# bobu36000/gym-chess

Hardware: AMD Instinct MI355X
Metric: env steps/sec at 65 536 boards per GPU (random-policy self-play to terminal, auto-reset) (higher is better)
Workload: dtype u64

## Files before the change

### __graft_entry__.py

```python
import os
import subprocess
import sys

ROOT = os.path.dirname(os.path.abspath(__file__))
PKG_DIR = os.path.join(ROOT, "gym-chess_amd")
LIB = os.path.join(PKG_DIR, "gym_chess_amd", "libgymchess.so")
CORE_HOST = os.path.join(ROOT, "tests", "core_host")


def _run(cmd):
    print("+", " ".join(cmd), flush=True)
    subprocess.run(cmd, check=True)


def _lib_module():
    sys.path.insert(0, PKG_DIR)
    from gym_chess_amd import _lib

    return _lib


def build_hip(force=False):
    L = _lib_module()
    want = L.source_hash()
    if not force and os.path.exists(LIB) and L.built_hash(LIB) == want:
        return
    tmp = LIB + ".tmp"
    _run(["hipcc"] + L.BUILD_FLAGS + [f'-DGC_SRC_HASH="{want}"', "-o", tmp,
                                      os.path.join(PKG_DIR, "csrc", "gymchess.hip")])
    os.replace(tmp, LIB)


def build_oracle():
    _run(["make", "-s", "-C", os.path.join(ROOT, "oracle")])


def build_core_host():
    sys.path.insert(0, CORE_HOST)
    import applysplithost
    import clonehost
    import corehost
    import minimaxhost
    import playouthost
    import quiescehost
    import rankfillhost
    import sworiginhost

    corehost.ensure_built()
    sworiginhost.ensure_built()
    rankfillhost.ensure_built()
    clonehost.ensure_built()
    applysplithost.ensure_built()
    playouthost.ensure_built()
    minimaxhost.ensure_built()
    quiescehost.ensure_built()


def build():
    build_hip()
    build_oracle()
    build_core_host()
    sys.path.insert(0, PKG_DIR)
    import gym_chess_amd
    from gym_chess_amd import _lib

    _lib.load()


def smoke():
    sys.path.insert(0, PKG_DIR)
    sys.path.insert(0, os.path.join(ROOT, "oracle"))
    import numpy as np

    import oracle as O
    from gym_chess_amd.engine import Engine
    from gym_chess_amd.env import BatchedChessEnv

    eng = Engine(0)
    b = np.tile(O.DEFAULT_BOARD, (64, 1))
    m = np.tile(O.make_meta(), (64, 1))
    nodes = eng.perft(b, m, 3)
    assert (nodes == 8982).all(), nodes[:4]
    moves, cnt = eng.possible_moves(b[:1], m[:1], True)
    assert [int(x) for x in moves[0, : cnt[0]]] == O.get_possible_moves(O.DEFAULT_BOARD, O.make_meta(), True)
    env = BatchedChessEnv(32, device=0, seed=7)
    _, tr = env.rollout(60, trace=True)
    for i in range(32):
        ref = O.rollout_trace(7, i, 60)
        assert (tr["action"][:, i] == ref["action"]).all(), f"board {i} actions differ"
        assert (tr["reward"][:, i] == ref["reward"]).all(), f"board {i} rewards differ"
        assert (tr["done"][:, i] == ref["done"]).all(), f"board {i} done differs"
    print("smoke ok: perft(3)=8982 x64, startpos list, 32x60-ply rollout == oracle", flush=True)


if __name__ == "__main__":
    build()
    if len(sys.argv) > 1 and sys.argv[1] == "smoke":
        smoke()
```

### gym-chess_amd/csrc/gc_core.h

```cpp
#pragma once
#include <type_traits>
#include <stdint.h>

#if defined(__HIPCC__)
#include <hip/hip_runtime.h>
#define GC_HD __host__ __device__ __forceinline__
#define GC_HDM __host__ __device__ __forceinline__
#else
#define GC_HD static inline
#define GC_HDM inline
#endif

namespace gc {

typedef uint64_t u64;
typedef uint32_t u32;

enum { EMPTY = 0, KING = 1, QUEEN = 2, ROOK = 3, BISHOP = 4, KNIGHT = 5, PAWN = 6 };
enum { A_KSW = 4096, A_QSW = 4097, A_KSB = 4098, A_QSB = 4099, A_RESIGN = 4100, A_NONE = 0xFFFF };

enum : u32 {
    M_WHITE = 1u, M_WKC = 2u, M_WQC = 4u, M_BKC = 8u, M_BQC = 16u, M_RIGHTS = 30u,
    M_WCHK = 32u, M_BCHK = 64u, M_DONE = 128u,
    M_MC_SHIFT = 8, M_MC_MASK = 0xFFu << 8,
// ... 1047 lines not shown
        if (k >= cc) { k -= cc; v >>= w; base += w; }
    }
    return base;
}
GC_HD u64 fast_pawn_targets(const MoveSet& ms, int sq, bool white) {
    u64 m = bit(sq);
    u64 t1 = white ? ((ms.o1 & m) >> 8) : ((ms.o1 & m) << 8);
    u64 t2 = white ? ((ms.o2 & m) >> 16) : ((ms.o2 & m) << 16);
    u64 tl = white ? ((ms.ol & m) >> 7) : ((ms.ol & m) << 9);
    u64 tr = white ? ((ms.orr & m) >> 9) : ((ms.orr & m) << 7);
    return t1 | t2 | tl | tr;
}
template <class S>
GC_HD int select_action(const Pos& s, const Gen& g, const MoveSet& ms, const S& scr, int k) {
    int normal = ms.total - popc(g.castles);
    if (k >= normal) {
        k -= normal;
        if (g.castles & 2) { if (k == 0) return g.white ? A_KSW : A_KSB; k--; }
        return g.white ? A_QSW : A_QSB;
    }
    if (ms.big) {
        u64 pcs = g.own;
        while (pcs) {
            int sq = ctz(pcs);
            pcs ^= bit(sq);
            u64 tg = legal_targets(s, g, sq, type_at(s, sq));
            int c = popc(tg);
            if (k < c) return sq * 64 + kth_set_bit(tg, k);
            k -= c;
        }
        return A_NONE;
    }
    int lo = 0, pre = 0;
#pragma unroll
    for (int step = 32; step; step >>= 1) {
        int p = prefix_count(ms.cnt, below(lo + step));
        bool take = p <= k;
        lo = take ? lo + step : lo;
        pre = take ? p : pre;
    }
    k -= pre;
    u64 parked = scr.get(ordinal(g.own, lo));
    u64 tg = ((ms.fastp >> lo) & 1) ? fast_pawn_targets(ms, lo, g.white) : parked;
    return lo * 64 + kth_set_bit(tg, k);
}

GC_HD u64 byte_popc(u64 x) {
    x = x - ((x >> 1) & 0x5555555555555555ull);
    x = (x & 0x3333333333333333ull) + ((x >> 2) & 0x3333333333333333ull);
    return (x + (x >> 4)) & 0x0F0F0F0F0F0F0F0Full;
}
GC_HD u64 spread8(u32 b) {
    u64 y = ((u64)(b & 0xFFu) * 0x0101010101010101ull) & 0x8040201008040201ull;
    return ((y + 0x7F7F7F7F7F7F7F7Full) >> 7) & 0x0101010101010101ull;
}
GC_HD int first_byte_above(u64 p, int k) {
    int r = (int)((p >> 24) & 0xFF) <= k ? 4 : 0;
    r += (int)((p >> (8 * r + 8)) & 0xFF) <= k ? 2 : 0;
    r += (int)((p >> (8 * r)) & 0xFF) <= k ? 1 : 0;
    return r;
}
template <class S>
GC_HD int select_action_swar(const Pos& s, const Gen& g, const MoveSet& ms, const S& scr, int k) {
    const int normal = ms.total - popc(g.castles);
    if (k >= normal || ms.big || normal > 255) return select_action(s, g, ms, scr, k);
    const u64 rows = byte_popc(ms.cnt[0]) + (byte_popc(ms.cnt[1]) << 1) + (byte_popc(ms.cnt[2]) << 2) +
                     (byte_popc(ms.cnt[3]) << 3) + (byte_popc(ms.cnt[4]) << 4);
    const u64 rpre = rows * 0x0101010101010101ull;
    const int r = first_byte_above(rpre, k);
    k -= r ? (int)((rpre >> (8 * r - 8)) & 0xFF) : 0;
    const int sh = 8 * r;
    const u64 sqs = spread8((u32)(ms.cnt[0] >> sh)) + (spread8((u32)(ms.cnt[1] >> sh)) << 1) +
                    (spread8((u32)(ms.cnt[2] >> sh)) << 2) + (spread8((u32)(ms.cnt[3] >> sh)) << 3) +
                    (spread8((u32)(ms.cnt[4] >> sh)) << 4);
    const u64 spre = sqs * 0x0101010101010101ull;
    const int f = first_byte_above(spre, k);
    k -= f ? (int)((spre >> (8 * f - 8)) & 0xFF) : 0;
    const int lo = sh + f;
    u64 parked = scr.get(ordinal(g.own, lo));
    u64 tg = ((ms.fastp >> lo) & 1) ? fast_pawn_targets(ms, lo, g.white) : parked;
    return lo * 64 + kth_set_bit(tg, k);
}

GC_HD int sw_origin(const Gen& g, int j, int to) {
    const u64 w0 = g.white ? pack8(8, 16, 7, 9, -15, -17, 17, 15) : pack8(-8, -16, -9, -7, -15, -17, 17, 15);
    const u64 w1 = pack8(-6, -10, 10, 6, 0, 0, 0, 0), w2 = pack8(0, 0, 0, 0, 8, -8, 1, -1);
    const u64 w3 = pack8(9, 7, -7, -9, 0, 0, 0, 0);
    const int q = j >> 3;
    const u64 w = q == 0 ? w0 : q == 1 ? w1 : q == 2 ? w2 : w3;
    const int off = (int)(signed char)(w >> (8 * (j & 7)));
    const int d = (j - SW_ORTH) & 7;
    const bool up = ((0xC6u >> d) & 1) != 0;
    const bool file = d < 2, row = d < 4, dg = d == 5 || d == 6;
    const u64 pl = file ? 0x0080808080808080ull : row ? 0x7FFFFFFFFFFFFFFFull : dg ? 0x0040201008040201ull : 0x0102040810204081ull;
    const u64 ph = file ? 0x0101010101010100ull : row ? 0xFFFFFFFFFFFFFFFEull : dg ? 0x8040201008040200ull : 0x8102040810204080ull;
    const u64 x = g.occ & (up ? pl >> (63 - to) : ph << to);
    const int sl = x ? (up ? msb(x) : ctz(x)) : 0;
    const bool slider = j >= SW_ORTH && j < SW_K;
    return slider ? sl : to + off;
}
GC_HD int sw_select(const Gen& g, const u64* t, int k) {
    int j = SW_SETS;
    u64 tj = 0;
#pragma unroll
    for (int i = 0; i < SW_SETS; i++) {
        const int c = popc(t[i]);
        const bool hit = j == SW_SETS && k < c;
        j = hit ? i : j;
        tj = hit ? t[i] : tj;
        k = j == SW_SETS ? k - c : k;
    }
    if (j == SW_SETS) {
        if ((g.castles & 1) && k == 0) return g.white ? A_QSW : A_QSB;
        return g.white ? A_KSW : A_KSB;
    }
    const int to = kth_set_bit(tj, k);
    return sw_origin(g, j, to) * 64 + to;
}

GC_HD void sw_pack(const u64* t, int lo, int hi, u64* cw) {
    for (int i = lo; i < hi; i++) cw[i >> 3] |= (u64)popc(t[i]) << (8 * (i & 7));
}
GC_HD u64 byte_prefix(u64 w) {
    w += w << 8;
    w += w << 16;
    return w + (w << 32);
}
GC_HD int sw_locate_pre(const u64* pw, int& k) {
    const u64 p0 = pw[0], p1 = pw[1], p2 = pw[2], p3 = pw[3];
    const int c1 = (int)(p0 >> 56), c2 = c1 + (int)(p1 >> 56), c3 = c2 + (int)(p2 >> 56);
    const int w = (k >= c1) + (k >= c2) + (k >= c3);
    const u64 p = w == 0 ? p0 : w == 1 ? p1 : w == 2 ? p2 : p3;
    k -= w == 0 ? 0 : w == 1 ? c1 : w == 2 ? c2 : c3;
    const u64 H = 0x8000800080008000ull, K = (u64)(k + 1) * 0x0001000100010001ull, M = 0x00FF00FF00FF00FFull;
    const int above = popc((((p & M) | H) - K) & H) + popc(((((p >> 8) & M) | H) - K) & H);
    const int b = 8 - above;
    k -= b ? (int)((p >> (8 * b - 8)) & 0xFF) : 0;
    return 8 * w + b;
}
GC_HD int sw_locate(const u64* cw, int& k) {
    const u64 pw[4] = {byte_prefix(cw[0]), byte_prefix(cw[1]), byte_prefix(cw[2]), byte_prefix(cw[3])};
    return sw_locate_pre(pw, k);
}
GC_HD int sw_finish(const Gen& g, int j, u64 tj, int k) {
    const int to = kth_set_bit(tj, k);
    return sw_origin(g, j, to) * 64 + to;
}
GC_HD int sw_castle(const Gen& g, int k) {
    if ((g.castles & 1) && k == 0) return g.white ? A_QSW : A_QSB;
    return g.white ? A_KSW : A_KSB;
}

template <class S>
GC_HD int select_move(const Pos& s, const Gen& g, const MoveSet& ms, const S& scr, int k) {
    if (ms.big) return select_legal(s, g, k);
    u64 t[SCRATCH_SLOTS];
#pragma unroll
    for (int j = 0; j < SCRATCH_SLOTS; j++) t[j] = scr.get(j);
#if defined(__HIP_DEVICE_COMPILE__)
#pragma unroll
    for (int j = 0; j < SCRATCH_SLOTS; j++) asm volatile("" : "+v"(t[j]));
#endif
    u64 pcs = g.own;
    int res = -1, rsq = 0, rk = 0;
    u64 rtg = 0;
    bool pawn = false;
#pragma unroll
    for (int j = 0; j < SCRATCH_SLOTS; j++) {
        bool live = pcs != 0 && res < 0;
        int sq = pcs ? ctz(pcs) : 0;
        pcs &= pcs - 1;
        bool fast = (ms.fastp >> sq) & 1;
        int pc = (int)(((ms.o1 >> sq) & 1) + ((ms.o2 >> sq) & 1) + ((ms.ol >> sq) & 1) + ((ms.orr >> sq) & 1));
        int c = fast ? pc : popc(t[j]);
        bool hit = live && k < c;
        res = hit ? j : res;
        rsq = hit ? sq : rsq;
        rk = hit ? k : rk;
        rtg = hit ? t[j] : rtg;
        pawn = hit ? fast : pawn;
        k = (live && !hit) ? k - c : k;
    }
    if (res >= 0) {
        int sq = rsq;
        k = rk;
        if (pawn) {
            if ((ms.o1 >> sq) & 1) { if (k == 0) return sq * 64 + (g.white ? sq - 8 : sq + 8); k--; }
            if ((ms.o2 >> sq) & 1) { if (k == 0) return sq * 64 + (g.white ? sq - 16 : sq + 16); k--; }
            if ((ms.ol >> sq) & 1) { if (k == 0) return sq * 64 + (g.white ? sq - 7 : sq + 9); k--; }
            return sq * 64 + (g.white ? sq - 9 : sq + 7);
        }
        return sq * 64 + kth_target(rtg, sq, type_at(s, sq), g.white, k);
    }
    if (g.castles & 1) { if (k == 0) return g.white ? A_QSW : A_QSB; k--; }
    if (g.castles & 2) { if (k == 0) return g.white ? A_KSW : A_KSB; }
    return A_NONE;
}

GC_HD bool action_legal(const Pos& s, const Gen& g, int action) {
    if (action < 0 || action > A_RESIGN) return false;
    if (action >= 4096) {
        if (g.white) return (action == A_QSW && (g.castles & 1)) || (action == A_KSW && (g.castles & 2));
        return (action == A_QSB && (g.castles & 1)) || (action == A_KSB && (g.castles & 2));
    }
    int f = action >> 6, t = action & 63;
    if (!((g.own >> f) & 1)) return false;
    return (legal_targets(s, g, f, type_at(s, f)) >> t) & 1;
}

GC_HD bool quick_legal(const Pos& s, int action) {
    if (action < 0 || action > A_RESIGN) return false;
    Gen g;
    gen_base(s, g);
    if (action >= 4096) {
        gen_enemy(s, g);
        return action_legal(s, g, action);
    }
    const int f = action >> 6, t = action & 63;
    if (!((g.own >> f) & 1)) return false;
    const int ty = type_at(s, f);
    if (ty == KING) return ((king_set(bit(f)) & ~g.own) >> t & 1) && !sq_attacked(s, t, !g.white);
    gen_pins(s, g);
    return (legal_targets(s, g, f, ty) >> t) & 1;
}

GC_HD bool quick_pseudo(const Pos& s, int action) {
    if (action < 0 || action > A_RESIGN) return false;
    Gen g;
    gen_base(s, g);
    if (action >= 4096) {
        gen_enemy(s, g);
        return action_legal(s, g, action);
    }
// ... 203 lines not shown
```

### gym-chess_amd/csrc/gc_quad.h

```cpp
#pragma once

#define QUAD_BOARDS 64
#ifndef QUADS_WG
#define QUADS_WG 2
#endif
#ifndef GC_QXOR
#define GC_QXOR 2
#endif
#define ROLL_QUADS_WG 1

struct QuadLds {
    u64 sets[SW_SETS][QUAD_BOARDS];
    u64 ns[NBB][QUAD_BOARDS];
    u32 nmeta[QUAD_BOARDS];
    int32_t mr[QUAD_BOARDS];
    u32 irrev[QUAD_BOARDS];
    u64 pin3[3][QUAD_BOARDS];
    u32 f0[QUAD_BOARDS];
    u64 enemy[3][QUAD_BOARDS];
    u32 f1[QUAD_BOARDS];
    u64 cw3[QUAD_BOARDS];
    u64 cw0[2][QUAD_BOARDS];
    u32 part[4][QUAD_BOARDS];
    u32 rep[QUAD_BOARDS];
    u32 x0[QUAD_BOARDS];
    u32 ra[QUAD_BOARDS];
    u32 act[QUAD_BOARDS];
    u32 pick[QUAD_BOARDS];
    u32 d[QUAD_BOARDS];
    u32 castles[QUAD_BOARDS];
    u64 occ[HTAB / 64][QUAD_BOARDS];
    u32 nkey[QUAD_BOARDS];
    u32 rkey0;
    Pos rp;
};
template <class LT>
struct QuadSetsT {
    LT& L;
    int l;
    u64 cw[4];
    int part;
    __device__ void put(int j, u64 t) {
        L.sets[j][l] = t;
        const int c = popc(t);
        cw[j >> 3] |= (u64)c << (8 * (j & 7));
        part += c;
    }
    template <int LO, int HI>
    __device__ void put_all(const u64* t) {
#pragma unroll
        for (int j = LO; j < HI; j++) put(j, t[j - LO]);
    }
};
using QuadSets = QuadSetsT<QuadLds>;

struct QuadPend {
    bool have;
    uint16_t ra;
    __device__ int resolve(const QuadLds& L, int l) const {
        const int pk = (int)L.pick[l];
        return have ? pk : (int)ra;
    }
};
struct QuadQ0Pre {
    u32 meta0;
    u64 occ, kw, rw;
};
template <bool S0>
__device__ __forceinline__ QuadQ0Pre quad_q0pre(const Pos& s) {
    QuadQ0Pre q{(s.meta & ~(u32)M_RIGHTS) | eff_rights(s), S0 ? 0ull : occ_of(s), s.k & s.w, s.r & s.w};
    pin(q.meta0); pin(q.kw); pin(q.rw);
    if (!S0) pin(q.occ);
    return q;
}
__device__ __forceinline__ QuadQ0Pre quad_q1pre(const Pos& s) {
    QuadQ0Pre q{0u, occ_of(s), 0ull, 0ull};
    pin(q.occ);
    return q;
}
struct QuadAhead {
    u32 x0, ra;
};
__device__ __forceinline__ void quad_ahead(const PairCtx& C, int i, u32 d, QuadAhead& ah) {
    ah.x0 = philox_x0(C.seed, (u32)i, d);
    ah.ra = C.rtable ? (u32)C.racts[scale_rank(ah.x0, C.rtotal)] : (u32)(uint16_t)A_NONE;
}

struct OccQ {
    bool valid;
    bool clr;
    bool probe;
    bool fast;
};
#ifndef GC_WG_FAIR
#define GC_WG_FAIR 1
#endif
#ifndef GC_OCC_RUN
#define GC_OCC_RUN 1
#endif
#define QSETPRIO(x, up)                                       \
    do {                                                      \
        if (GC_WG_FAIR && (up)) __builtin_amdgcn_s_setprio((x) + 1); \
        else __builtin_amdgcn_s_setprio(x);                   \
    } while (0)
template <int R, bool OCC, bool S0>
__device__ __forceinline__ StepOut quad_ply(QuadLds& L, const PairCtx& C, int l, int i, bool live, Pos& s, int& a,
                                            u32& d, DevHist& h, u32& nst, RepProbe& pr, QuadPend& pend, OccQ& oq,
                                            QuadQ0Pre& q0, QuadAhead& ah, bool up = false) {
    constexpr bool CARRY = R < 2;
#ifdef GC_PSTAMPS
    bool pst_loaded = false;
#endif
    if (R == 0) QSETPRIO(2, up);
    if (R == 2) QSETPRIO(0, up);
    if (GC_WG_FAIR && R == 1) QSETPRIO(2, up);
    if (GC_WG_FAIR && R == 3) QSETPRIO(0, up);
    if (R == 0 || (S0 && R == 1)) a = pend.resolve(L, l);
    u32 x0 = 0;
    uint16_t ra = (uint16_t)A_NONE;
    if (R == 1 && !S0) {
        x0 = philox_x0(C.seed, (u32)i, d);
        if (C.rtable) ra = C.racts[scale_rank(x0, C.rtotal)];
        L.x0[l] = x0;
    }
    if (R == 3 && S0) {
        const u32 dt = L.d[l];
        if (__any(dt != d)) {
            d = dt;
            quad_ahead(C, i, d, ah);
        }
        L.x0[l] = ah.x0;
        L.ra[l] = ah.ra;
    }
    if (R == 0 && !S0) L.act[l] = (u32)a;
    PST(7);
    if (R == 1 && !S0) {
        pair_barrier();
        a = (int)L.act[l];
    }
    const bool none = a == A_NONE;
    const bool done0 = (s.meta & M_DONE) != 0;
    const bool cap = mc_of(s.meta) > MOVES_MAX;
    const bool mv = live && !none && !done0 && !cap;
    const bool white = (s.meta & M_WHITE) != 0;
// ... 27 lines not shown
        if (!mv) {
        } else if (cas) {
            apply_legal_with(ns, white, a, &mr, &irrev, q0.occ, q0.kw, q0.rw);
        } else {
            apply_legal_with<false>(ns, white, a, &mr, &irrev, q0.occ, q0.kw, q0.rw);
        }
        L.ns[0][l] = ns.k; L.ns[1][l] = ns.q; L.ns[2][l] = ns.r; L.ns[3][l] = ns.b;
        L.ns[4][l] = ns.n; L.ns[5][l] = ns.p; L.ns[6][l] = ns.w;
        L.nmeta[l] = ns.meta;
        L.mr[l] = mr;
        L.irrev[l] = irrev ? 1u : 0u;
    }
    PST(0);
    if (S0) PST_ARRIVE(0);
    if (R != 1 || S0) pair_barrier();
    if (S0) PST_LAST(0);
    PST(1);
    Gen g;
    bool my_chk = false;
    OrthCarry oc{};
    DiagCarry dc{};
    if (R == 0 && S0) {
        ns.q = L.ns[1][l]; ns.b = L.ns[3][l]; ns.n = L.ns[4][l]; ns.p = L.ns[5][l];
    } else if (R == 1 && S0) {
        ns.k = L.ns[0][l]; ns.r = L.ns[2][l]; ns.w = L.ns[6][l];
        ns.meta = L.nmeta[l];
    } else if (R != 0) {
        ns.k = L.ns[0][l]; ns.q = L.ns[1][l]; ns.r = L.ns[2][l]; ns.b = L.ns[3][l];
        ns.n = L.ns[4][l]; ns.p = L.ns[5][l]; ns.w = L.ns[6][l];
        ns.meta = L.nmeta[l];
    }
    if (R == 1 && !S0) {
        mr = L.mr[l];
        irrev = L.irrev[l] != 0;
    }
    gen_base(ns, g);
    if (R == 0) {
        gen_pins(ns, g);
        L.pin3[0][l] = g.checkmask;
        L.pin3[1][l] = g.pinned;
        L.pin3[2][l] = g.pinrays;
        L.f0[l] = g.in_check ? 1u : 0u;
    } else if (R == 1) {
        my_chk = mv && mover_checked(s, ns, white, a);
        L.f1[l] = my_chk ? 1u : 0u;
        if constexpr (OCC) {
        if (oq.clr) {
#pragma unroll
            for (int w = 0; w < HTAB / 64; w++) L.occ[w][l] = 0ull;
            oq.clr = false;
        }
        const u32 nk = board_key(ns);
        L.nkey[l] = nk;
        oq.probe = !oq.valid || ((L.occ[(nk & (HTAB - 1)) >> 6][l] >> (nk & 63)) & 1) != 0;
        }
    } else if (R == 2) {
        oc = orth_carry(g.occ);
        L.enemy[1][l] = g.ks >= 0 ? side_attacks_leapers(ns, !g.white) | side_attacks_orth(ns, !g.white, oc) : 0ull;
    } else {
        dc = diag_carry(g.occ);
        L.enemy[2][l] = g.ks >= 0 ? side_attacks_diag(ns, !g.white, dc) : 0ull;
    }
    PST(2);
    if (S0) PST_ARRIVE(1);
    pair_barrier();
    if (S0) PST_LAST(1);
    PST(3);
#define QUAD_ENEMY(l) (L.enemy[1][l] | L.enemy[2][l])
    if (R == 0) {
        g.enemy_att = QUAD_ENEMY(l);
        gen_castles(ns, g);
        my_chk = L.f1[l] != 0;
    } else if (R == 1) {
        g.in_check = L.f0[l] != 0;
    } else {
        g.checkmask = L.pin3[0][l];
        g.pinned = L.pin3[1][l];
        g.pinrays = L.pin3[2][l];
        if (R == 2) g.enemy_att = QUAD_ENEMY(l);
    }
    const bool opp_chk = g.in_check;
    const bool both = opp_chk && my_chk;
    const bool gen = mv && !both;
    QuadSets Q{L, l, {0, 0, 0, 0}, 0};
    int c = 0;
    u32 hl = hl_of(s.meta);
    if (R == 0) {
        if (gen) {
            u64 T[SW_SETS];
            sw_pawns(ns, g, T);
            Q.put_all<SW_P1, SW_N>(T + SW_P1);
            sw_knights(ns, g, T);
            Q.put_all<SW_N, SW_ORTH>(T + SW_N);
            Q.part += popc(g.castles);
        }
        L.cw0[0][l] = byte_prefix(Q.cw[0]);
        L.cw0[1][l] = byte_prefix(Q.cw[1]);
        L.castles[l] = g.castles;
    } else if (R == 1) {
        if (mv && !both) {
            pin(pr.e0.hdr); pin(pr.e0.k); pin(pr.e0.q); pin(pr.e0.r);
            pin(pr.e0.b); pin(pr.e0.n); pin(pr.e0.p); pin(pr.e0.w);
            if (OCC && oq.fast) pr.e0.hdr = (u64)(h.gen() ^ 1u);
            if constexpr (OCC && GC_OCC_RUN) {
                c = rep_commit(h, s, pr, hl, irrev, [&](u32 pos) {
                    const bool free = oq.valid && ((L.occ[pos >> 6][l] >> (pos & 63)) & 1) == 0;
                    PST_LOADED(!free);
                    return free;
                });
            } else {
                c = rep_commit(h, s, pr, hl, irrev, [&](u32) {
                    PST_LOADED(true);
                    return false;
                });
            }
            if (!OCC) {
            } else if (irrev) {
                oq.valid = true;
                oq.clr = true;
                oq.probe = false;
            } else if (h.wkind == 2) {
                L.occ[h.wpos >> 6][l] |= 1ull << (h.wpos & 63);
                oq.probe = oq.probe || (u32)h.wpos == (L.nkey[l] & (HTAB - 1));
            }
        }
        L.rep[l] = (u32)c | (hl << 8);
        if (!S0) L.ra[l] = ra;
    } else if (R == 2) {
        u64 T[SW_SETS];
        sw_orth(ns, g, oc, T);
        Q.put_all<SW_ORTH, SW_DIAG>(T + SW_ORTH);
        sw_kings(ns, g, T);
        Q.put_all<SW_K, SW_SETS>(T + SW_K);
        L.part[2][l] = (u32)Q.part;
#pragma unroll
        for (int k = 1; k < 4; k++) Q.cw[k] = byte_prefix(Q.cw[k]);
    } else {
        u64 T[SW_SETS];
        sw_diag(ns, g, dc, T);
        Q.put_all<SW_DIAG, SW_K>(T + SW_DIAG);
        L.part[3][l] = (u32)Q.part;
        L.cw3[l] = byte_prefix(Q.cw[2]);
    }
    if (R == 0) L.part[0][l] = (u32)Q.part;
#ifdef GC_PSTAMPS
    if (R == 1) gc_pst_mark_run(4, pst_loaded);
    else
#endif
    PST(4);
    if (S0) PST_ARRIVE(2);
    pair_barrier();
    if (S0) PST_LAST(2);
    PST(5);
    StepOut o = {0, 0, R_NONE, 0};
    if (R == 0) QSETPRIO(0, up);
    if (R == 2) QSETPRIO(2, up);
    if (R == 2) {
        const int total = (int)L.part[0][l] + Q.part + (int)L.part[3][l];
        const u64 cw[4] = {L.cw0[0][l], Q.cw[1] + L.cw0[1][l], Q.cw[2] + L.cw3[l], Q.cw[3]};
        g.castles = L.castles[l];
        L.pick[l] = total > 0 ? (u32)sw_pick_lds<true>(L, l, g, cw, total, (int)scale_rank(L.x0[l], (u32)total)) : (u32)A_NONE;
    }
    if constexpr (CARRY) {
        const int total = gen ? (R == 0 ? Q.part : (int)L.part[0][l]) + (int)L.part[2][l] + (int)L.part[3][l] : 0;
        if (R == 0) {
            const u32 rpk = L.rep[l];
            c = (int)(rpk & 0xFFu);
            hl = rpk >> 8;
            ra = (uint16_t)L.ra[l];
        } else {
            if (S0) ra = (uint16_t)L.ra[l];
            h.commit();
        }
        bool have = false;
        if (none) {
            o.reason = R_NO_MOVES;
        } else {
            nst += 1;
            if (done0) { o.done = 1; o.reason = R_DONE_ALREADY; }
            else if (cap) { o.done = 1; o.reason = R_MOVE_CAP; }
            else if (both) { o.done = 1; o.reason = R_BOTH_CHECKED; }
            else {
                const u32 chk = white ? ((my_chk ? M_WCHK : 0u) | (opp_chk ? M_BCHK : 0u))
                                      : ((opp_chk ? M_WCHK : 0u) | (my_chk ? M_BCHK : 0u));
                s = ns;
                s.meta = with_hl((ns.meta & ~(u32)(M_WCHK | M_BCHK | M_DONE)) | chk | ((c >= 3 || c == 0) ? M_DONE : 0u), hl);
                o.reward = -10 + mr;
                o.moved = 1;
                if (c >= 3) { o.done = 1; o.reason = R_REPETITION; }
                if (c == 0) { o.done = 1; o.reason = R_WINDOW_FULL; }
                if (total == 0 && opp_chk) {
                    s.meta |= M_DONE;
                    o.done = 1;
                    o.reward += 100;
                    o.reason = R_MATE;
                }
                if (!o.done && !white) s.meta += (1u << M_MC_SHIFT);
                have = true;
            }
            if (o.done) have = false;
        }
        if (!have) {
            s = L.rp;
            h.bump_gen();
        }
        if (R == 1 && OCC) {
            pr.key = have ? L.nkey[l] : L.rkey0;
            if (!have) {
                oq.valid = true;
                oq.clr = true;
            }
            oq.fast = !(live && have && oq.probe);
            const ulonglong2* src = oq.fast ? reinterpret_cast<const ulonglong2*>(C.icd)
                                            : reinterpret_cast<const ulonglong2*>(h.htab + h.entry((int)(pr.key & (HTAB - 1))) * 8);
            const ulonglong2 e0 = src[0], e1 = src[1], e2 = src[2], e3 = src[3];
            pr.e0 = RepEntry{e0.x, e0.y, e1.x, e1.y, e2.x, e2.y, e3.x, e3.y};
        } else if (R == 1 && live) {
            rep_prefetch(h, s, pr);
        }
        const int tot = have ? total : (int)C.rtotal;
        d += tot > 0 ? 1u : 0u;
        if (R == 0) {
            if (S0) L.d[l] = d;
            pend = QuadPend{have, ra};
            q0 = quad_q0pre<S0>(s);
        } else if (S0) {
            pend = QuadPend{have, ra};
            q0 = quad_q1pre(s);
        }
    }
    if (R == 3 && S0) {
        d += 1u;
        pin(d);
        quad_ahead(C, i, d, ah);
    }
    PST(6);
    if (S0) PST_ARRIVE(3);
    pair_barrier();
    if (S0) PST_LAST(3);
    return o;
}

__shared__ QuadLds g_quad_lds[ROLL_QUADS_WG];
__shared__ QuadLds g_quad_lds2[QUADS_WG];
template <int QW>
__device__ __forceinline__ QuadLds& roll_lds(int qw) {
    if constexpr (QW == ROLL_QUADS_WG) return g_quad_lds[qw];
    else return g_quad_lds2[qw];
}

#define ROLL_TURNS 0xCA69C6A9C69AC69Cull
template <int QW>
__device__ __forceinline__ int roll_place(int block, int wgs) {
    const int part = wgs / (4 / QW);
    return (part ? block / part : block) & (4 / QW - 1);
}
template <int QW>
__device__ __forceinline__ bool roll_turn(int place, int turn) {
    if (QW == 2) return ((place ^ turn) & 1) != 0;
    return ((ROLL_TURNS >> (4 * (turn & 15) + place)) & 1) != 0;
}

template <int RR, bool ST, bool OCC, int QW>
__device__ __forceinline__ void quad_run(uint8_t* __restrict__ slab, int nn, uint64_t seed, u64* __restrict__ htab,
                                      const uint16_t* __restrict__ racts, const EnvDev::InitCache* __restrict__ icd,
                                      u32 rinfo, int plies, uint64_t* __restrict__ stats, u64* __restrict__ trace,
                                      int qw, int l, int i, int place) {
    constexpr bool S0 = QW == ROLL_QUADS_WG;
    QuadLds& L = roll_lds<QW>(qw);
    const bool live = i < nn;
    const int ii = live ? i : nn - 1;
    const PairIO in_io(slab, nn);
    const PairCtx C = {seed, htab, in_io.hgen, racts, icd, (rinfo >> 16) != 0, rinfo & 0xFFFFu};
    Pos s{};
    u32 ua = 0, g0 = 0, nst = 0, d = 0;
    if (RR == 3 && S0) {
        d = in_io.draw[ii];
        pin(d);
    }
    if (RR < 2) {
        s = in_io.load(ii);
        ua = in_io.act[ii];
        g0 = in_io.hgen[ii];
        nst = in_io.nsteps[ii];
// ... 216 lines not shown
```

### gym-chess_amd/csrc/gymchess.hip

```cpp
#include <hip/hip_runtime.h>
#include <hipcub/hipcub.hpp>

#include <cmath>
#include <cstdio>
#include <cstdlib>
#include <cstring>
#include <atomic>
#include <chrono>
#include <mutex>
#include <string>
#include <type_traits>
#include <vector>

#include "gc_stamps.h"
#include "gc_core.h"
#include "gc_env.h"
#include "gc_perft.h"
#include "gc_fide.h"
#include "gc_policy.h"
#include "gc_priors.h"
#include "../../include/gymchess.h"

using namespace gc;
namespace gcf = gc::fide;
// ... 1042 lines not shown
                }
            }
        } else {
            if (gen) part = ms.big ? count_legal(ns, g) : gen_moves_a(ns, g, ms, scr) + popc(g.castles);
        }
    } else {
        if constexpr (SW) {
            constexpr int W1_TO = SW_K;
            u64 cw[4] = {0, 0, 0, 0};
            if (gen) {
                if constexpr (FIDE) {
                    gcf::fsw_gen_b(ns, gcf::FGen{g, 0, -1}, H.T);
                } else {
                    sw_orth(ns, g, H.T);
                    sw_diag_part<0, 4>(ns, g, H.T);
                }
                sw_pack(H.T, SW_ORTH, W1_TO, cw);
                part = sw_popc(H.T, SW_ORTH, W1_TO);
#pragma unroll
                for (int j = SW_ORTH; j < W1_TO; j++) L.sets[j][l] = H.T[j];
            }
            L.swc[0][l] = cw[1];
            L.swc[1][l] = cw[2];
        } else if (gen && !ms.big) {
            part = FIDE ? gen_moves_b<PairScratch, true>(ns, g, ms, scr) : gen_moves_b(ns, g, ms, scr);
        }
        if (mv && !both) {
            pin(pr.e0.hdr); pin(pr.e0.k); pin(pr.e0.q); pin(pr.e0.r);
            pin(pr.e0.b); pin(pr.e0.n); pin(pr.e0.p); pin(pr.e0.w);
            c = rep_commit(h, s, pr, hl, irrev);
        }
        L.rep[l] = (u32)c | (hl << 8);
        w1_late();
    }
    if constexpr (!SW) {
#pragma unroll
        for (int b = 0; b < 5; b++) L.planes[role][b][l] = ms.cnt[b];
    }
    L.part[role][l] = (u32)part;
    GC_STAMP(4);
    PST(4);
    pair_barrier();
    PST(5);
    GC_STAMP(5);

    if constexpr (SW) {
        if (role == 0) {
            H.cw[1] |= L.swc[0][l];
            H.cw[2] |= L.swc[1][l];
        }
    } else {
#pragma unroll
        for (int b = 0; b < 5; b++) ms.cnt[b] |= L.planes[role ^ 1][b][l];
    }
    ms.total = part + (int)L.part[role ^ 1][l];
    if (role == 0) {
        u32 rpk = L.rep[l];
        c = (int)(rpk & 0xFFu);
        hl = rpk >> 8;
    }
    H.ns = ns;
    H.mr = mr;
    H.irrev = irrev;
    H.my_chk = my_chk;
    H.opp_chk = opp_chk;
    H.both = both;
    H.mv = mv;
    H.c = c;
    H.hl = hl;
    H.ep_from = ep_from;
    H.ep = ep;
}

__device__ __forceinline__ Pos pair_settle(const PairHalf& H, bool white) {
    u32 chk = white ? ((H.my_chk ? M_WCHK : 0u) | (H.opp_chk ? M_BCHK : 0u))
                    : ((H.opp_chk ? M_WCHK : 0u) | (H.my_chk ? M_BCHK : 0u));
    Pos ns = H.ns;
    ns.meta = with_hl((ns.meta & ~(u32)(M_WCHK | M_BCHK | M_DONE)) | chk | ((H.c >= 3 || H.c == 0) ? M_DONE : 0u), H.hl);
    return ns;
}

template <bool PRE = false, class LdsT>
__device__ __forceinline__ int sw_pick_lds(const LdsT& L, int l, const Gen& g, const u64* cw, int tot, int k) {
    const int normal = tot - popc(g.castles);
    int r = k, j;
    if (tot < 256) {
        j = PRE ? sw_locate_pre(cw, r) : sw_locate(cw, r);
    } else {
#pragma unroll 1
        for (j = 0; j < SW_SETS - 1; j++) {
            const int c = popc(L.sets[j][l]);
            if (r < c) break;
            r -= c;
        }
    }
    j = j < SW_SETS ? j : SW_SETS - 1;
    const int set_act = sw_finish(g, j, L.sets[j][l], r);
    return k >= normal ? sw_castle(g, k - normal) : set_act;
}

template <bool SHARE_ACT, bool FIDE = false, class RT = int>
__device__ __forceinline__ StepOut pair_ply(PairLds& L, const PairCtx& C, RT role, int l, int i,
                                            bool live, const Pos& rp, Pos& s, int& a, u32& d, DevHist& h,
                                            u32& nst) {
    constexpr bool SW = true;
    const bool none = a == A_NONE;
    const bool done0 = (s.meta & M_DONE) != 0;
    const bool cap = mc_of(s.meta) > MOVES_MAX;
    const bool mv = live && !none && !done0 && !cap;
    const bool white = (s.meta & M_WHITE) != 0;
    u32 x0 = 0;
    uint16_t ra = (uint16_t)A_NONE;
    PairHalf H;
    pair_half<FIDE, false, false, SW>(
        L, role, l, mv, false, s, a, nullptr, nullptr, h, H,
        [&] {
            x0 = philox_x0(C.seed, (u32)i, d);
            if (C.rtable) ra = C.racts[scale_rank(x0, C.rtotal)];
            L.x0[l] = x0;
        },
        [&] { L.ra[l] = ra; });
    if (role == 0) {
        x0 = L.x0[l];
        ra = (uint16_t)L.ra[l];
    }
    else h.commit();
    Gen& g = H.g;
    MoveSet& ms = H.ms;
    int set_act = A_NONE;
    if (role == 0 && ms.total > 0) set_act = sw_pick_lds(L, l, g, H.cw, ms.total, (int)scale_rank(x0, (u32)ms.total));
    StepOut o = {0, 0, R_NONE, 0};
    bool have = false;
    if (none) {
        o.reason = R_NO_MOVES;
    } else {
        nst += 1;
        if (done0) { o.done = 1; o.reason = R_DONE_ALREADY; }
        else if (cap) { o.done = 1; o.reason = R_MOVE_CAP; }
        else if (H.both) { o.done = 1; o.reason = R_BOTH_CHECKED; }
        else {
            s = pair_settle(H, white);
            o.reward = -10 + H.mr;
            o.moved = 1;
            if (H.c >= 3) { o.done = 1; o.reason = R_REPETITION; }
            if (H.c == 0) { o.done = 1; o.reason = R_WINDOW_FULL; }
            if (ms.total == 0 && H.opp_chk) {
                s.meta |= M_DONE;
                o.done = 1;
                o.reward += 100;
                o.reason = R_MATE;
            }
            if (!o.done && !white) s.meta += (1u << M_MC_SHIFT);
            have = true;
        }
        if (o.done) have = false;
    }
    if (!have) {
        s = rp;
        h.bump_gen();
    }
    if (role == 0) {
        uint16_t act = (uint16_t)set_act;
        int tot = ms.total;
        if (!have && C.rtable) {
            act = ra;
            tot = (int)C.rtotal;
        } else if (!have) {
            if constexpr (FIDE) {
                gcf::FGen fr;
                gcf::fgen(s, fr);
                g = fr.g;
                tot = gcf::fsw_gen(s, fr, H.T);
            } else {
                gen_init(s, g);
                tot = sw_gen(s, g, H.T);
            }
            H.cw[0] = H.cw[1] = H.cw[2] = H.cw[3] = 0;
            sw_pack(H.T, 0, SW_SETS, H.cw);
#pragma unroll
            for (int j = 0; j < SW_SETS; j++) L.sets[j][l] = H.T[j];
            act = (uint16_t)(tot > 0 ? sw_pick_lds(L, l, g, H.cw, tot, (int)scale_rank(x0, (u32)tot)) : A_NONE);
// ... 2147 lines not shown
```

Baseline: 20.21 billion.

## Streamline sliding-origin lookup, fused count prefix, and branchless quad ply outcome

Rewrites sw_origin to use a bit-reversed occupancy so both ray directions share one ctz path. Builds per-lane byte-prefix count words directly from popcounts instead of packing and then prefix-summing. Makes the quad-ply terminal/outcome logic branchless. Wraps the slow >=256 selection loop behind a wave-uniform __any check so the common path avoids divergence. Together these aim to cut ALU and divergence in the per-ply move selection, at the cost of extra bit-reverse instructions and compiler-pinning asm hints.

```diff
diff --git a/__graft_entry__.py b/__graft_entry__.py
--- a/__graft_entry__.py
+++ b/__graft_entry__.py
@@ -40,6 +40,7 @@
     import applysplithost
     import clonehost
     import corehost
+    import countprefixhost
     import minimaxhost
     import playouthost
     import quiescehost
@@ -54,6 +55,7 @@
     playouthost.ensure_built()
     minimaxhost.ensure_built()
     quiescehost.ensure_built()
+    countprefixhost.ensure_built()
 
 
 def build():
diff --git a/gym-chess_amd/csrc/gc_core.h b/gym-chess_amd/csrc/gc_core.h
--- a/gym-chess_amd/csrc/gc_core.h
+++ b/gym-chess_amd/csrc/gc_core.h
@@ -1153,20 +1153,28 @@
     return lo * 64 + kth_set_bit(tg, k);
 }
 
+GC_HD u64 brev64(u64 x) {
+#if defined(__HIP_DEVICE_COMPILE__)
+    return __brevll(x);
+#else
+    x = ((x >> 1) & 0x5555555555555555ull) | ((x & 0x5555555555555555ull) << 1);
+    x = ((x >> 2) & 0x3333333333333333ull) | ((x & 0x3333333333333333ull) << 2);
+    x = ((x >> 4) & 0x0F0F0F0F0F0F0F0Full) | ((x & 0x0F0F0F0F0F0F0F0Full) << 4);
+    return __builtin_bswap64(x);
+#endif
+}
 GC_HD int sw_origin(const Gen& g, int j, int to) {
-    const u64 w0 = g.white ? pack8(8, 16, 7, 9, -15, -17, 17, 15) : pack8(-8, -16, -9, -7, -15, -17, 17, 15);
-    const u64 w1 = pack8(-6, -10, 10, 6, 0, 0, 0, 0), w2 = pack8(0, 0, 0, 0, 8, -8, 1, -1);
-    const u64 w3 = pack8(9, 7, -7, -9, 0, 0, 0, 0);
-    const int q = j >> 3;
-    const u64 w = q == 0 ? w0 : q == 1 ? w1 : q == 2 ? w2 : w3;
-    const int off = (int)(signed char)(w >> (8 * (j & 7)));
-    const int d = (j - SW_ORTH) & 7;
-    const bool up = ((0xC6u >> d) & 1) != 0;
+    const u32 pw = g.white ? (u32)(pack8(0, 0, 0, 0, 8, 16, 7, 9) >> 32) : (u32)(pack8(0, 0, 0, 0, -8, -16, -9, -7) >> 32);
+    const u64 nw = pack8(-15, -17, 17, 15, -6, -10, 10, 6), kw = pack8(8, -8, 1, -1, 9, 7, -7, -9);
+    const u32 d = ((u32)j + 4u) & 7u;
+    const u64 w = j < SW_N ? (u64)pw << 32 : j < SW_ORTH ? nw : kw;
+    const int off = (int)(signed char)(w >> (8 * d));
+    const u32 flip = ((0xC6u >> d) & 1u) ? 63u : 0u;
     const bool file = d < 2, row = d < 4, dg = d == 5 || d == 6;
-    const u64 pl = file ? 0x0080808080808080ull : row ? 0x7FFFFFFFFFFFFFFFull : dg ? 0x0040201008040201ull : 0x0102040810204081ull;
     const u64 ph = file ? 0x0101010101010100ull : row ? 0xFFFFFFFFFFFFFFFEull : dg ? 0x8040201008040200ull : 0x8102040810204080ull;
-    const u64 x = g.occ & (up ? pl >> (63 - to) : ph << to);
-    const int sl = x ? (up ? msb(x) : ctz(x)) : 0;
+    const u64 o = flip ? brev64(g.occ) : g.occ;
+    const u64 x = o & (ph << ((u32)to ^ flip));
+    const int sl = x ? (int)((u32)ctz(x | (1ull << 63)) ^ flip) : 0;
     const bool slider = j >= SW_ORTH && j < SW_K;
     return slider ? sl : to + off;
 }
@@ -1199,15 +1207,45 @@
 }
 GC_HD int sw_locate_pre(const u64* pw, int& k) {
     const u64 p0 = pw[0], p1 = pw[1], p2 = pw[2], p3 = pw[3];
-    const int c1 = (int)(p0 >> 56), c2 = c1 + (int)(p1 >> 56), c3 = c2 + (int)(p2 >> 56);
-    const int w = (k >= c1) + (k >= c2) + (k >= c3);
+    const u32 c1 = (u32)(p0 >> 56), c2 = c1 + (u32)(p1 >> 56), c3 = c2 + (u32)(p2 >> 56);
+    const u32 uk = (u32)k;
+    const u32 w = (uk >= c1 ? 1u : 0u) + (uk >= c2 ? 1u : 0u) + (uk >= c3 ? 1u : 0u);
     const u64 p = w == 0 ? p0 : w == 1 ? p1 : w == 2 ? p2 : p3;
-    k -= w == 0 ? 0 : w == 1 ? c1 : w == 2 ? c2 : c3;
-    const u64 H = 0x8000800080008000ull, K = (u64)(k + 1) * 0x0001000100010001ull, M = 0x00FF00FF00FF00FFull;
-    const int above = popc((((p & M) | H) - K) & H) + popc(((((p >> 8) & M) | H) - K) & H);
-    const int b = 8 - above;
-    k -= b ? (int)((p >> (8 * b - 8)) & 0xFF) : 0;
-    return 8 * w + b;
+    u32 r = uk - (w == 0 ? 0u : w == 1 ? c1 : w == 2 ? c2 : c3);
+    const u32 H = 0x80008000u, K = (r + 1u) | ((r + 1u) << 16), M = 0x00FF00FFu;
+    const u32 pl = (u32)p, ph = (u32)(p >> 32);
+    const u32 above = (u32)__builtin_popcount((((pl & M) | H) - K) & H) + (u32)__builtin_popcount(((((pl >> 8) & M) | H) - K) & H) +
+                      (u32)__builtin_popcount((((ph & M) | H) - K) & H) + (u32)__builtin_popcount(((((ph >> 8) & M) | H) - K) & H);
+    const u32 b = 8u - above;
+    r -= b ? (u32)((p >> (8u * b - 8u)) & 0xFFu) : 0u;
+    k = (int)r;
+    return (int)(8u * w + b);
+}
+enum : u32 { SW_OWN_Q0 = 0x0000FFFu, SW_OWN_Q2 = 0xFF0F000u, SW_OWN_Q3 = 0x00F0000u };
+template <u32 OWN>
+GC_HD void sw_prefix_make(const u64* t, u64* pw, u32& part) {
+    part = 0;
+#pragma unroll
+    for (int w = 0; w < 4; w++) {
+        u32 run = 0, h[2] = {0, 0};
+#pragma unroll
+        for (int b = 0; b < 8; b++) {
+            const int j = 8 * w + b;
+            if (j < SW_SETS && ((OWN >> j) & 1u)) {
+                run += (u32)__builtin_popcount((u32)t[j]);
+#if defined(__HIP_DEVICE_COMPILE__)
+                asm("" : "+v"(run));
+#endif
+                run += (u32)__builtin_popcount((u32)(t[j] >> 32));
+#if defined(__HIP_DEVICE_COMPILE__)
+                asm("" : "+v"(run));
+#endif
+            }
+            h[b >> 2] |= run << (8 * (b & 3));
+        }
+        pw[w] = (u64)h[0] | ((u64)h[1] << 32);
+        part += run;
+    }
 }
 GC_HD int sw_locate(const u64* cw, int& k) {
     const u64 pw[4] = {byte_prefix(cw[0]), byte_prefix(cw[1]), byte_prefix(cw[2]), byte_prefix(cw[3])};
@@ -1220,6 +1258,28 @@
 GC_HD int sw_castle(const Gen& g, int k) {
     if ((g.castles & 1) && k == 0) return g.white ? A_QSW : A_QSB;
     return g.white ? A_KSW : A_KSB;
+}
+template <bool PRE, class GetSet>
+GC_HD int sw_pick_sets(const GetSet& get, const Gen& g, const u64* cw, int tot, int k, bool any_big) {
+    const int normal = tot - popc(g.castles);
+    int r = k, j = PRE ? sw_locate_pre(cw, r) : sw_locate(cw, r);
+#if defined(__HIP_DEVICE_COMPILE__)
+    asm volatile("" : "+v"(j), "+v"(r));
+#endif
+    if (any_big) {
+        if (tot >= 256) {
+            r = k;
+#pragma unroll 1
+            for (j = 0; j < SW_SETS - 1; j++) {
+                const int c = popc(get(j));
+                if (r < c) break;
+                r -= c;
+            }
+        }
+    }
+    j = j < SW_SETS ? j : SW_SETS - 1;
+    const int set_act = sw_finish(g, j, get(j), r);
+    return k >= normal ? sw_castle(g, k - normal) : set_act;
 }
 
 template <class S>
diff --git a/gym-chess_amd/csrc/gc_quad.h b/gym-chess_amd/csrc/gc_quad.h
--- a/gym-chess_amd/csrc/gc_quad.h
+++ b/gym-chess_amd/csrc/gc_quad.h
@@ -52,14 +52,19 @@
         for (int j = LO; j < HI; j++) put(j, t[j - LO]);
     }
 };
-using QuadSets = QuadSetsT<QuadLds>;
+template <int LO, int HI>
+__device__ __forceinline__ void quad_put(QuadLds& L, int l, const u64* t) {
+#pragma unroll
+    for (int j = LO; j < HI; j++) L.sets[j][l] = t[j];
+}
 
 struct QuadPend {
     bool have;
     uint16_t ra;
     __device__ int resolve(const QuadLds& L, int l) const {
-        const int pk = (int)L.pick[l];
-        return have ? pk : (int)ra;
+        u32 pk = L.pick[l];
+        pin(pk);
+        return have ? (int)pk : (int)ra;
     }
 };
 struct QuadQ0Pre {
@@ -253,20 +258,22 @@
     const bool opp_chk = g.in_check;
     const bool both = opp_chk && my_chk;
     const bool gen = mv && !both;
-    QuadSets Q{L, l, {0, 0, 0, 0}, 0};
+    u64 pw[4] = {0, 0, 0, 0};
+    u32 part = 0;
     int c = 0;
     u32 hl = hl_of(s.meta);
     if (R == 0) {
         if (gen) {
             u64 T[SW_SETS];
             sw_pawns(ns, g, T);
-            Q.put_all<SW_P1, SW_N>(T + SW_P1);
+            quad_put<SW_P1, SW_N>(L, l, T);
             sw_knights(ns, g, T);
-            Q.put_all<SW_N, SW_ORTH>(T + SW_N);
-            Q.part += popc(g.castles);
-        }
-        L.cw0[0][l] = byte_prefix(Q.cw[0]);
-        L.cw0[1][l] = byte_prefix(Q.cw[1]);
+            quad_put<SW_N, SW_ORTH>(L, l, T);
+            sw_prefix_make<SW_OWN_Q0>(T, pw, part);
+            part += (u32)popc(g.castles);
+        }
+        L.cw0[0][l] = pw[0];
+        L.cw0[1][l] = pw[1];
         L.castles[l] = g.castles;
     } else if (R == 1) {
         if (mv && !both) {
@@ -300,20 +307,21 @@
     } else if (R == 2) {
         u64 T[SW_SETS];
         sw_orth(ns, g, oc, T);
-        Q.put_all<SW_ORTH, SW_DIAG>(T + SW_ORTH);
+        quad_put<SW_ORTH, SW_DIAG>(L, l, T);
         sw_kings(ns, g, T);
-        Q.put_all<SW_K, SW_SETS>(T + SW_K);
-        L.part[2][l] = (u32)Q.part;
-#pragma unroll
-        for (int k = 1; k < 4; k++) Q.cw[k] = byte_prefix(Q.cw[k]);
+        quad_put<SW_K, SW_SETS>(L, l, T);
+        sw_prefix_make<SW_OWN_Q2>(T, pw, part);
+        L.part[2][l] = part;
+        pin(pw[1]); pin(pw[2]); pin(pw[3]);
     } else {
         u64 T[SW_SETS];
         sw_diag(ns, g, dc, T);
-        Q.put_all<SW_DIAG, SW_K>(T + SW_DIAG);
-        L.part[3][l] = (u32)Q.part;
-        L.cw3[l] = byte_prefix(Q.cw[2]);
-    }
-    if (R == 0) L.part[0][l] = (u32)Q.part;
+        quad_put<SW_DIAG, SW_K>(L, l, T);
+        sw_prefix_make<SW_OWN_Q3>(T, pw, part);
+        L.part[3][l] = part;
+        L.cw3[l] = pw[2];
+    }
+    if (R == 0) L.part[0][l] = part;
 #ifdef GC_PSTAMPS
     if (R == 1) gc_pst_mark_run(4, pst_loaded);
     else
@@ -327,13 +335,13 @@
     if (R == 0) QSETPRIO(0, up);
     if (R == 2) QSETPRIO(2, up);
     if (R == 2) {
-        const int total = (int)L.part[0][l] + Q.part + (int)L.part[3][l];
-        const u64 cw[4] = {L.cw0[0][l], Q.cw[1] + L.cw0[1][l], Q.cw[2] + L.cw3[l], Q.cw[3]};
+        const int total = (int)L.part[0][l] + (int)part + (int)L.part[3][l];
+        const u64 cw[4] = {L.cw0[0][l], pw[1] + L.cw0[1][l], pw[2] + L.cw3[l], pw[3]};
         g.castles = L.castles[l];
         L.pick[l] = total > 0 ? (u32)sw_pick_lds<true>(L, l, g, cw, total, (int)scale_rank(L.x0[l], (u32)total)) : (u32)A_NONE;
     }
     if constexpr (CARRY) {
-        const int total = gen ? (R == 0 ? Q.part : (int)L.part[0][l]) + (int)L.part[2][l] + (int)L.part[3][l] : 0;
+        const int total = gen ? (R == 0 ? (int)part : (int)L.part[0][l]) + (int)L.part[2][l] + (int)L.part[3][l] : 0;
         if (R == 0) {
             const u32 rpk = L.rep[l];
             c = (int)(rpk & 0xFFu);
@@ -343,34 +351,23 @@
             if (S0) ra = (uint16_t)L.ra[l];
             h.commit();
         }
-        bool have = false;
-        if (none) {
-            o.reason = R_NO_MOVES;
-        } else {
-            nst += 1;
-            if (done0) { o.done = 1; o.reason = R_DONE_ALREADY; }
-            else if (cap) { o.done = 1; o.reason = R_MOVE_CAP; }
-            else if (both) { o.done = 1; o.reason = R_BOTH_CHECKED; }
-            else {
-                const u32 chk = white ? ((my_chk ? M_WCHK : 0u) | (opp_chk ? M_BCHK : 0u))
-                                      : ((opp_chk ? M_WCHK : 0u) | (my_chk ? M_BCHK : 0u));
-                s = ns;
-                s.meta = with_hl((ns.meta & ~(u32)(M_WCHK | M_BCHK | M_DONE)) | chk | ((c >= 3 || c == 0) ? M_DONE : 0u), hl);
-                o.reward = -10 + mr;
-                o.moved = 1;
-                if (c >= 3) { o.done = 1; o.reason = R_REPETITION; }
-                if (c == 0) { o.done = 1; o.reason = R_WINDOW_FULL; }
-                if (total == 0 && opp_chk) {
-                    s.meta |= M_DONE;
-                    o.done = 1;
-                    o.reward += 100;
-                    o.reason = R_MATE;
-                }
-                if (!o.done && !white) s.meta += (1u << M_MC_SHIFT);
-                have = true;
-            }
-            if (o.done) have = false;
-        }
+        const bool play = !none && !done0 && !cap && !both;
+        const bool rep3 = c >= 3, full = c == 0, mate = total == 0 && opp_chk;
+        const bool end1 = rep3 || full || mate;
+        const u32 chk = white ? ((my_chk ? M_WCHK : 0u) | (opp_chk ? M_BCHK : 0u))
+                              : ((opp_chk ? M_WCHK : 0u) | (my_chk ? M_BCHK : 0u));
+        u32 meta1 = with_hl((ns.meta & ~(u32)(M_WCHK | M_BCHK | M_DONE)) | chk | ((rep3 || full) ? M_DONE : 0u), hl);
+        meta1 |= mate ? (u32)M_DONE : 0u;
+        meta1 += !end1 && !white ? (1u << M_MC_SHIFT) : 0u;
+        const int reason1 = mate ? R_MATE : full ? R_WINDOW_FULL : rep3 ? R_REPETITION : R_NONE;
+        const bool have = play && !end1;
+        nst += none ? 0u : 1u;
+        o.reward = play ? -10 + mr + (mate ? 100 : 0) : 0;
+        o.done = none ? 0 : play ? (end1 ? 1 : 0) : 1;
+        o.reason = none ? R_NO_MOVES : done0 ? R_DONE_ALREADY : cap ? R_MOVE_CAP : both ? R_BOTH_CHECKED : reason1;
+        o.moved = play ? 1 : 0;
+        s = ns;
+        s.meta = meta1;
         if (!have) {
             s = L.rp;
             h.bump_gen();
diff --git a/gym-chess_amd/csrc/gymchess.hip b/gym-chess_amd/csrc/gymchess.hip
--- a/gym-chess_amd/csrc/gymchess.hip
+++ b/gym-chess_amd/csrc/gymchess.hip
@@ -1148,21 +1148,7 @@
 
 template <bool PRE = false, class LdsT>
 __device__ __forceinline__ int sw_pick_lds(const LdsT& L, int l, const Gen& g, const u64* cw, int tot, int k) {
-    const int normal = tot - popc(g.castles);
-    int r = k, j;
-    if (tot < 256) {
-        j = PRE ? sw_locate_pre(cw, r) : sw_locate(cw, r);
-    } else {
-#pragma unroll 1
-        for (j = 0; j < SW_SETS - 1; j++) {
-            const int c = popc(L.sets[j][l]);
-            if (r < c) break;
-            r -= c;
-        }
-    }
-    j = j < SW_SETS ? j : SW_SETS - 1;
-    const int set_act = sw_finish(g, j, L.sets[j][l], r);
-    return k >= normal ? sw_castle(g, k - normal) : set_act;
+    return sw_pick_sets<PRE>([&](int j) { return L.sets[j][l]; }, g, cw, tot, k, __any(tot >= 256) != 0);
 }
 
 template <bool SHARE_ACT, bool FIDE = false, class RT = int>
```

Result: faster. 20.57 billion (median of 6 runs) (+1.8%).
